# marcin-ochman/modular-slam

Hardware: AMD Instinct MI355X
Metric: ORB keypoints extracted+matched /sec, 640×480 RGB-D, 1/2/4/8 GPU; HBM GB/s vs roofline (higher is better)
Workload: dtype u8

## Files before the change

### include/mslam_hip.h

```cpp
#ifndef MSLAM_HIP_H_
#define MSLAM_HIP_H_

#include <stddef.h>
#include <stdint.h>

#ifdef __cplusplus
extern "C" {
#endif

#define MSLAM_HIP_ABI_VERSION 5

enum
{
    MSLAM_HIP_OK = 0,
    MSLAM_HIP_E_INVALID = 1,
    MSLAM_HIP_E_RUNTIME = 2,
    MSLAM_HIP_E_CAPACITY = 3,
    MSLAM_HIP_E_NO_VOCABULARY = 4,
    MSLAM_HIP_E_FORMAT = 5,
    MSLAM_HIP_E_NO_MODEL = 6
};

typedef struct mslam_hip_ctx mslam_hip_ctx;

// ... 412 lines not shown
                               const double* tvec, int min_matched_points, int new_keyframe_min_landmarks, int new_id,
                               double z_max, mslam_hip_track_window_result* out , int* first_event,
                               int32_t* vote_counts, int32_t* entry_src, int32_t* entry_kp, int entry_capacity);

#define MSLAM_HIP_TSDF_CHUNK 64
#define MSLAM_HIP_TSDF_MAX_VOXELS (1 << 30)
#define MSLAM_HIP_TSDF_MAX_FRAMES 32768
typedef struct
{
    int32_t nx, ny, nz;
    int32_t max_frames;
    double voxel;
    double origin[3];
    double trunc;
    double max_depth;
    int32_t width, height;
    float factor;
    int32_t reserved;
    double fx, fy, cx, cy;
} mslam_hip_tsdf_params;
int mslam_hip_tsdf_create(mslam_hip_ctx* ctx, const mslam_hip_tsdf_params* params);
int mslam_hip_tsdf_destroy(mslam_hip_ctx* ctx);
int mslam_hip_tsdf_info(mslam_hip_ctx* ctx, mslam_hip_tsdf_params* out , int* n_frames );
int mslam_hip_tsdf_add_frame(mslam_hip_ctx* ctx, int frame_id, const uint16_t* depth, const double* R, const double* t);
int mslam_hip_tsdf_add_frame_dev(mslam_hip_ctx* ctx, int frame_id, const uint16_t* d_depth, const double* R, const double* t);
int mslam_hip_tsdf_get_frame(mslam_hip_ctx* ctx, int frame_id, double* R, double* t);
int mslam_hip_tsdf_update_poses(mslam_hip_ctx* ctx, const int32_t* frame_ids, const double* R ,
                                const double* t , int n, int* n_moved);
int mslam_hip_tsdf_remove_frame(mslam_hip_ctx* ctx, int frame_id);
int mslam_hip_tsdf_read(mslam_hip_ctx* ctx, int32_t* S, int32_t* W);
int mslam_hip_tsdf_extract(mslam_hip_ctx* ctx, int min_weight, float* xyz, float* normal, int capacity, int* n);

typedef struct
{
    int32_t width, height;
    double fx, fy, cx, cy;
    double z_near, z_far, step;
    int32_t coarse;
    int32_t min_weight;
} mslam_hip_tsdf_raycast_params;
int mslam_hip_tsdf_raycast(mslam_hip_ctx* ctx, const mslam_hip_tsdf_raycast_params* params, const double* R, const double* t,
                           float* depth, float* xyz, float* normal, int* n_hits);
int mslam_hip_tsdf_raycast_dev(mslam_hip_ctx* ctx, const mslam_hip_tsdf_raycast_params* params, const double* R, const double* t,
                               float* d_depth, float* d_xyz, float* d_normal, int* n_hits);

enum
{
    MSLAM_HIP_DBG_PYRAMID = 0,
    MSLAM_HIP_DBG_BLURRED = 1,
    MSLAM_HIP_DBG_CANDIDATES = 2,
    MSLAM_HIP_DBG_SELECTED = 3,
    MSLAM_HIP_DBG_CELLS = 4,
    MSLAM_HIP_DBG_FORMS = 5,
    MSLAM_HIP_DBG_QUAD_DIRECT = 6
};
int mslam_hip_level_geometry(mslam_hip_ctx* ctx, int* widths, int* heights, float* scales);
int mslam_hip_debug_read(mslam_hip_ctx* ctx, int what, int frame, int level, void* dst, size_t dst_bytes,
                         size_t* n_items);

int mslam_hip_debug_counts(mslam_hip_ctx* ctx, int what, int32_t* out, int n_frames);

int mslam_hip_copy_to_host(mslam_hip_ctx* ctx, void* dst_host, const void* src_dev, size_t bytes);

int mslam_hip_set_profiling(mslam_hip_ctx* ctx, int enable);
int mslam_hip_get_stage_times(mslam_hip_ctx* ctx, const char** names, float* ms, int cap, int* n);

#ifdef __cplusplus
}
#endif
#endif
```

### modular-slam_amd/__init__.py

```python
import contextlib
import ctypes as C
import os
import subprocess

import numpy as np

_HERE = os.path.dirname(os.path.abspath(__file__))
LIB_PATH = os.path.join(_HERE, "libmslam_hip.so")

OK, E_INVALID, E_RUNTIME, E_CAPACITY, E_NO_VOCABULARY, E_FORMAT, E_NO_MODEL = range(7)
DBG_PYRAMID, DBG_BLURRED, DBG_CANDIDATES, DBG_SELECTED, DBG_CELLS, DBG_FORMS, DBG_QUAD_DIRECT = range(7)
QUAD_DIRECT_MAX_CANDIDATES = 1024
MATCHER_AUTO, MATCHER_POPCOUNT = 0, 1
DETECTOR_DISTRIBUTED, DETECTOR_CV_ORB = 0, 1
BOW_ASSIGN_TREE, BOW_ASSIGN_FLAT = 0, 1
CV_ORDER_LIBSTDCXX, CV_ORDER_RASTER = 0, 1
POSE_GRAPH_MAX_KEYFRAMES, POSE_GRAPH_MAX_EDGES = 1024, 65536
POSE_GRAPH_MAX_KEYFRAMES_SPARSE, POSE_GRAPH_MAX_ENVELOPE_BLOCKS = 16384, 1048576
PG_SOLVER_DENSE, PG_SOLVER_SPARSE = 0, 1
_PG_SOLVER_NAMES = {"dense": PG_SOLVER_DENSE, "sparse": PG_SOLVER_SPARSE}
PG_ORDER_NATURAL, PG_ORDER_RCM = 0, 1
BA_GLOBAL_MAX_KEYFRAMES, BA_GLOBAL_MAX_KEYFRAMES_SPARSE = 1024, 16384
BA_GLOBAL_SOLVER_DENSE, BA_GLOBAL_SOLVER_SPARSE = 0, 1
BA_GLOBAL_PCG_MAX_ITERATIONS, BA_GLOBAL_PCG_TOLERANCE = 500, 1e-6
POSE_GRAPH_PCG_MAX_ITERATIONS, POSE_GRAPH_PCG_TOLERANCE = 500, 1e-6
CULL_MAX_ENTRIES = 4096
BA_LOSS_NONE, BA_LOSS_HUBER, BA_LOSS_CAUCHY = 0, 1, 2
_BA_LOSS_NAMES = {"none": BA_LOSS_NONE, "huber": BA_LOSS_HUBER, "cauchy": BA_LOSS_CAUCHY}
UNION_DESC_RECENT, UNION_DESC_DISTINCTIVE = 0, 1
_UNION_DESC_NAMES = {"recent": UNION_DESC_RECENT, "distinctive": UNION_DESC_DISTINCTIVE}
TRACK_POSE_PNP, TRACK_POSE_ALIGN = 0, 1
_TRACK_POSE_NAMES = {"pnp": TRACK_POSE_PNP, "align": TRACK_POSE_ALIGN}
TSDF_CHUNK, TSDF_MAX_VOXELS, TSDF_MAX_FRAMES = 64, 1 << 30, 32768

ABI_SYMBOLS = [
    "mslam_hip_default_params", "mslam_hip_abi_version", "mslam_hip_create", "mslam_hip_destroy",
    "mslam_hip_last_error", "mslam_hip_sync", "mslam_hip_detect", "mslam_hip_detect_batch_dev",
    "mslam_hip_get_batch_view", "mslam_hip_match", "mslam_hip_match_knn2", "mslam_hip_match_batch_dev",
    "mslam_hip_bow_load", "mslam_hip_bow_info", "mslam_hip_bow_words", "mslam_hip_bow_transform",
    "mslam_hip_bow_score", "mslam_hip_bow_db_add", "mslam_hip_bow_db_query", "mslam_hip_bow_db_clear",
    "mslam_hip_bow_batch_dev", "mslam_hip_get_bow_view", "mslam_hip_bow_cross_score_dev", "mslam_hip_level_geometry", "mslam_hip_debug_read",
    "mslam_hip_set_profiling", "mslam_hip_get_stage_times", "mslam_hip_copy_to_host", "mslam_hip_backproject", "mslam_hip_backproject_batch_dev",
    "mslam_hip_get_points_view", "mslam_hip_set_matcher", "mslam_hip_get_matcher",
    "mslam_hip_bow_pack_dev", "mslam_hip_bow_cross_score_packed_dev", "mslam_hip_debug_counts",
    "mslam_hip_last_match_kernel",
    "mslam_hip_join_matcher", "mslam_hip_bow_db_remove", "mslam_hip_bow_set_assignment",
    "mslam_hip_bow_db_reserve", "mslam_hip_bow_db_size", "mslam_hip_qlz_decompress",
    "mslam_hip_pnp_ransac", "mslam_hip_pnp_batch_dev", "mslam_hip_get_pnp_view", "mslam_hip_pnp_set_confidence", "mslam_hip_pack_batch_dev", "mslam_hip_packed_capacity",
    "mslam_hip_set_cv_keypoint_order", "mslam_hip_pnp_min_mse", "mslam_hip_pnp_min_mse_batch_dev",
    "mslam_hip_kf_add", "mslam_hip_kf_add_from_batch_dev", "mslam_hip_kf_remove", "mslam_hip_kf_clear", "mslam_hip_kf_size",
    "mslam_hip_kf_reserve", "mslam_hip_kf_read", "mslam_hip_relocalize",
    "mslam_hip_kf_visible", "mslam_hip_track", "mslam_hip_track_window", "mslam_hip_track_window_dev",
    "mslam_hip_kf_add_ids", "mslam_hip_kf_read_ids", "mslam_hip_kf_covisible", "mslam_hip_kf_union", "mslam_hip_kf_union_dev",
    "mslam_hip_match_guided_knn2", "mslam_hip_match_guided", "mslam_hip_set_guided_match", "mslam_hip_get_guided_match",
    "mslam_hip_bundle_adjust", "mslam_hip_bundle_adjust_global", "mslam_hip_kf_update_world", "mslam_hip_pose_graph",
    "mslam_hip_kf_fuse_search", "mslam_hip_kf_replace_ids", "mslam_hip_kf_fuse",
    "mslam_hip_kf_fuse_search_multi", "mslam_hip_kf_fuse_multi",
    "mslam_hip_kf_remove_observations",
    "mslam_hip_kf_observers", "mslam_hip_kf_cull_search", "mslam_hip_kf_cull",
    "mslam_hip_kf_remove_landmarks", "mslam_hip_kf_cull_landmarks_search", "mslam_hip_kf_cull_landmarks",
    "mslam_hip_set_ba_loss", "mslam_hip_get_ba_loss",
    "mslam_hip_set_union_descriptor", "mslam_hip_get_union_descriptor",
    "mslam_hip_set_pose_graph_solver", "mslam_hip_get_pose_graph_solver", "mslam_hip_pose_graph_analyze",
    "mslam_hip_set_ba_global_solver", "mslam_hip_get_ba_global_solver", "mslam_hip_bundle_adjust_global_analyze",
    "mslam_hip_set_pose_graph_loss", "mslam_hip_get_pose_graph_loss", "mslam_hip_pose_graph_edge_weights",
# ... 1215 lines not shown
    def bow_pack_dev(self, k_max, d_out):
        self._chk(self.L.mslam_hip_bow_pack_dev(self._h, int(k_max), C.c_void_p(d_out)))

    def bow_cross_score_packed_dev(self, d_sets, n_sets, self_set, n_frames, k_max, d_scores, stream=None):
        self._chk(self.L.mslam_hip_bow_cross_score_packed_dev(self._h, C.c_void_p(d_sets), int(n_sets), int(self_set),
                                                              int(n_frames), int(k_max), C.c_void_p(d_scores),
                                                              C.c_void_p(stream)))

    def bow_view(self):
        v = BowView()
        self._chk(self.L.mslam_hip_get_bow_view(self._h, C.byref(v)))
        return v

    def level_geometry(self):
        n = self.params.n_levels
        w = (C.c_int * 16)()
        h = (C.c_int * 16)()
        s = (C.c_float * 16)()
        self._chk(self.L.mslam_hip_level_geometry(self._h, w, h, s))
        return list(w[:n]), list(h[:n]), np.array(s[:n], np.float32)

    def debug_image(self, what, frame, level):
        w, h, _ = self.level_geometry()
        out = np.empty((h[level], w[level]), np.uint8)
        n = C.c_size_t(0)
        self._chk(self.L.mslam_hip_debug_read(self._h, what, frame, level, _p(out), C.c_size_t(out.size), C.byref(n)))
        return out

    def debug_keypoints(self, what, frame, level):
        out = np.empty((self.params.max_candidates, 3), np.float32)
        n = C.c_size_t(0)
        self._chk(self.L.mslam_hip_debug_read(self._h, what, frame, level, _p(out), C.c_size_t(out.nbytes),
                                              C.byref(n)))
        return out[:n.value].copy()

    def debug_cells(self, level):
        out = np.empty((2048, 6), np.int32)
        n = C.c_size_t(0)
        self._chk(self.L.mslam_hip_debug_read(self._h, DBG_CELLS, 0, level, _p(out), C.c_size_t(out.nbytes),
                                              C.byref(n)))
        return out[:n.value].copy()

    def debug_forms(self):
        out = np.zeros(2, np.int32)
        n = C.c_size_t(0)
        self._chk(self.L.mslam_hip_debug_read(self._h, DBG_FORMS, 0, 0, _p(out), C.c_size_t(out.nbytes), C.byref(n)))
        return int(out[0]), int(out[1])

    def debug_quad_direct_levels(self):
        out = np.zeros(1, np.uint32)
        n = C.c_size_t(0)
        self._chk(self.L.mslam_hip_debug_read(self._h, DBG_QUAD_DIRECT, 0, 0, _p(out), C.c_size_t(out.nbytes), C.byref(n)))
        return [bool((int(out[0]) >> l) & 1) for l in range(self.params.n_levels)]

    def debug_counts(self, what, n_frames):
        out = np.zeros((max(n_frames, 1), self.params.n_levels), np.int32)
        self._chk(self.L.mslam_hip_debug_counts(self._h, int(what), _p(out), int(out.shape[0])))
        return out[:n_frames]

    def set_profiling(self, enable):
        self._chk(self.L.mslam_hip_set_profiling(self._h, int(enable)))

    def stage_times(self, cap=256):
        names = (C.c_char_p * cap)()
        ms = (C.c_float * cap)()
        n = C.c_int(0)
        self._chk(self.L.mslam_hip_get_stage_times(self._h, names, ms, cap, C.byref(n)))
        return [(names[i].decode(), ms[i]) for i in range(n.value)]


def qlz_decompress(data, n_packets, capacity=None):
    src = np.frombuffer(bytes(data), np.uint8)
    cap = capacity if capacity is not None else 10000 * n_packets + 16
    dst = np.empty(max(cap, 1), np.uint8)
    n = C.c_size_t(0)
    L = lib()
    L.mslam_hip_qlz_decompress.argtypes = [C.c_void_p, C.c_size_t, C.c_uint32, C.c_void_p, C.c_size_t, C.POINTER(C.c_size_t)]
    rc = L.mslam_hip_qlz_decompress(_p(src), src.size, int(n_packets), _p(dst), dst.size, C.byref(n))
    if rc != OK:
        raise MslamHipError(rc, "qlz_decompress failed")
    return dst[:n.value].tobytes()


class RgbFrame:

    def __init__(self, data, width, height):
        self.data = np.ascontiguousarray(data, np.uint8).reshape(height, width, 3)
        self.size = (width, height)


class OrbKeypoint:
    __slots__ = ("id", "coordinates", "descriptor")

    def __init__(self, id, coordinates, descriptor):
        self.id, self.coordinates, self.descriptor = id, coordinates, descriptor


class HipOrbDetector:

    def __init__(self, width=640, height=480, **kw):
        self.ctx = Context(width=width, height=height, **kw)

    def detect(self, sensorData):
        r = self.ctx.detect(sensorData.data)
        return [OrbKeypoint(i, (float(x), float(y)), d) for i, ((x, y), d) in enumerate(zip(r["xy"].astype(np.float64),
                                                                                          r["desc"]))]
# ... 953 lines not shown
```

### modular-slam_amd/csrc/api.hip

```cpp
#include "context.hpp"

#include <cfloat>
#include <climits>
#include <cmath>
#include <cstdio>
#include <cstring>
#include <cstdlib>
#include <algorithm>

using namespace mslam;

static thread_local std::string g_create_error;

#define ENTER(c)                                                                                                       \
    do                                                                                                                 \
    {                                                                                                                  \
        if(!(c))                                                                                                       \
            return MSLAM_HIP_E_INVALID;                                                                                \
        MSLAM_CHK(c, hipSetDevice((c)->p.device));                                                                     \
    } while(0)

static inline int cv_round_f(float v) { return (int)lrintf(v); }
static inline int cv_floor_f(float v)
{
// ... 621 lines not shown
            const char* k = getenv("MSLAM_HIP_LEVEL_K6");
            const char* ks = getenv("MSLAM_HIP_LEVEL_K6_SMALL");
            c->level_k6_small = ks ? std::max(0, atoi(ks)) : 0;
            {
                const char* lc = getenv("MSLAM_HIP_LEVEL_CHAIN");
                const char* lf = getenv("MSLAM_HIP_LEVEL_CHAIN_FRAMES");
                const char* lw = getenv("MSLAM_HIP_LEVEL_CHAIN_WAVES");
                const char* lk = getenv("MSLAM_HIP_LEVEL_CHAIN_K6");
                c->level_chain = lc ? atoi(lc) : 0;
                c->level_chain_frames = lf ? std::max(1, std::min(64, atoi(lf))) : 2;
                c->level_chain_waves = lw ? atoi(lw) : 8;
                if(c->level_chain_waves != 4)
                    c->level_chain_waves = 8;
                c->level_chain_k6 = lk ? std::max(1, std::min(9, atoi(lk))) : 9;
            }
            c->level_k6 = k ? std::max(1, atoi(k)) : 5;
            const bool fits = (p.width & 3) == 0 && (double)B * p.width * p.height * 3 < 4294967296.0 &&
                              (double)B * g.slab < 4294901760.0  && (size_t)B * (p.width / 4) < (1u << 22) && p.height >= 8;
            int n_fused = fits ? 1 : 0;
            while(n_fused >= 1 && n_fused < p.n_levels && c->rs_q[n_fused] != SIZE_MAX && g.lv[n_fused].h >= 8 &&
                  (size_t)B * ((g.lv[n_fused].w + 3) / 4) < (1u << 22))
                ++n_fused;
            c->fused_levels = std::max(0, std::min(want, n_fused));
            const char* t = getenv("MSLAM_HIP_TILED_BLUR");
            c->geom.blur_tiled = c->fused_levels == p.n_levels && !(t && atoi(t) == 0) ? 1 : 0;
        }
        std::vector<BlurWave> bw;
        build_blur_waves(g, c->fused_levels, bw);
        c->blur_wpf = (int)bw.size();
        if(!bw.empty())
        {
            MSLAM_CHK(c, c->d_blur_waves.alloc(bw.size()));
            MSLAM_CHK(c, hipMemcpy(c->d_blur_waves, bw.data(), bw.size() * sizeof(BlurWave), hipMemcpyHostToDevice));
        }
    }
    MSLAM_CHK(c, c->d_cell_cnt.alloc(B * g.n_cells));
    MSLAM_CHK(c, c->d_cell_kp.alloc(B * g.n_cells * (size_t)kCellCap));
    QuadArgs& q = c->quad;
    MSLAM_CHK(c, c->q_cand.alloc(B * L * cap));
    MSLAM_CHK(c, c->q_cand_cnt.alloc(B * L));
    MSLAM_CHK(c, c->q_sel.alloc(B * L * cap));
    MSLAM_CHK(c, c->q_sel_cnt.alloc(B * L));
    MSLAM_CHK(c, c->q_kp_node.alloc(B * L * cap));
    MSLAM_CHK(c, c->q_nodes_a.alloc(B * L * cap));
    MSLAM_CHK(c, c->q_nodes_b.alloc(B * L * cap));
    MSLAM_CHK(c, c->q_ncnt_a.alloc(B * L * cap));
    MSLAM_CHK(c, c->q_ncnt_b.alloc(B * L * cap));
    MSLAM_CHK(c, c->q_child_cnt.alloc(B * L * cap * 4));
    MSLAM_CHK(c, c->q_ninfo.alloc(B * L * cap));
    MSLAM_CHK(c, c->q_best.alloc(B * L * cap));
    q.cand = c->q_cand, q.cand_cnt = c->q_cand_cnt, q.sel = c->q_sel, q.sel_cnt = c->q_sel_cnt, q.kp_node = c->q_kp_node;
    q.nodes_a = c->q_nodes_a, q.nodes_b = c->q_nodes_b, q.ncnt_a = c->q_ncnt_a, q.ncnt_b = c->q_ncnt_b;
    q.child_cnt = c->q_child_cnt, q.ninfo = c->q_ninfo, q.best = c->q_best;
    q.cell_cnt = c->d_cell_cnt;
    q.cell_kp = c->d_cell_kp;
    q.flags = c->d_flags;
    q.cand_cap = p.max_candidates;
    q.min_size = p.min_node_area;
    }

    for(auto& o : c->out)
    {
        MSLAM_CHK(c, o.xy.alloc((B + 1) * K * 2));
        MSLAM_CHK(c, o.desc.alloc((B + 1) * K * 32));
        MSLAM_CHK(c, o.octave.alloc((B + 1) * K));
        MSLAM_CHK(c, o.angle.alloc((B + 1) * K));
        MSLAM_CHK(c, o.response.alloc((B + 1) * K));
        MSLAM_CHK(c, o.count.alloc(B + 1));
        MSLAM_CHK(c, hipMemset(o.count, 0, (B + 1) * 4));
        MSLAM_CHK(c, o.idx0.alloc(B * K));
        MSLAM_CHK(c, o.idx1.alloc(B * K));
        MSLAM_CHK(c, o.dist0.alloc(B * K));
        MSLAM_CHK(c, o.dist1.alloc(B * K));
        MSLAM_CHK(c, o.mfrom.alloc(B * K));
        MSLAM_CHK(c, o.mto.alloc(B * K));
        MSLAM_CHK(c, o.mcount.alloc(B));
        MSLAM_CHK(c, hipMemset(o.mcount, 0, B * 4));
        MSLAM_CHK(c, hipEventCreateWithFlags(&o.ev_detect, hipEventDisableTiming));
        MSLAM_CHK(c, hipEventCreateWithFlags(&o.ev_match, hipEventDisableTiming));
    }
    MSLAM_CHK(c, hipStreamCreateWithFlags(&c->stream_m, hipStreamNonBlocking));
    {
        const char* e = getenv("MSLAM_HIP_OVERLAP_MATCH");
        c->overlap_match = !(e && atoi(e) == 0);
        auto on = [](const char* name) { const char* v = getenv(name); return !v || atoi(v) != 0; };
        c->knob_mirror_results = on("MSLAM_HIP_MIRROR_RESULTS");
        c->knob_zero_copy = on("MSLAM_HIP_ZERO_COPY_FRAME");
        c->knob_match_graph = on("MSLAM_HIP_MATCH_GRAPH");
        const char* zm = getenv("MSLAM_HIP_ZERO_COPY_MAX_BYTES");
        c->zero_copy_max_bytes = zm ? (size_t)atoll(zm) : (size_t)1200000;
        const char* m = getenv("MSLAM_HIP_MATCHER");
        c->matcher_kind = (m && std::strcmp(m, "popcount") == 0) ? MSLAM_HIP_MATCHER_POPCOUNT : MSLAM_HIP_MATCHER_AUTO;
    }
    c->cur = 0;
    MSLAM_CHK(c, hipDeviceSynchronize());
    return MSLAM_HIP_OK;
}

int mslam_hip_create(const mslam_hip_params* p, mslam_hip_ctx** out)
{
    if(!p || !out)
    {
        g_create_error = "null argument";
        return MSLAM_HIP_E_INVALID;
    }
    *out = nullptr;
// ... 261 lines not shown
                if(l < c->fused_levels)
                {
                    enqueue_resize_blur(c, l, c->d_rs_ofs + c->rs_y[l], c->d_rs_coef + c->rs_y[l], 0, f0, nf, k6_batch, cs);
                    continue;
                }
                if(c->rs_q[l] != SIZE_MAX)
                {
                    const LevelGeom &sl = g.lv[l - 1], &dl = g.lv[l];
                    ResizeColArgs ra{};
                    ra.pyr = c->d_pyr;
                    ra.slab = g.slab;
                    ra.src_off = sl.offset;
                    ra.sh = sl.h;
                    ra.spitch = sl.pitch;
                    ra.dst_off = dl.offset;
                    ra.dw = dl.w;
                    ra.dh = dl.h;
                    ra.dpitch = dl.pitch;
                    ra.qt = c->d_rs_qt + 3 * c->rs_q[l];
                    ra.yofs = c->d_rs_ofs + c->rs_y[l];
                    ra.ycoef = c->d_rs_coef + c->rs_y[l];
                    ra.frame0 = f0;
                    ra.n_frames = nf;
                    ra.quads = (dl.w + 3) / 4;
                    ra.inv_quads = 1.0f / (float)ra.quads;
                    ra.R = 8;
                    ra.need_mask = c->rs_need[l];
                    launch_resize_col(ra, cs);
                }
                else
                    launch_resize(c->d_pyr, g, l, c->d_rs_ofs + c->rs_x[l], c->d_rs_coef + c->rs_x[l],
                                  c->d_rs_ofs + c->rs_y[l], c->d_rs_coef + c->rs_y[l], f0, nf, cs);
            }
        }
        {
            StageScope t(c, "fast", cs);
            launch_fast(c->d_pyr, g, c->d_cells, c->d_cell_cnt, c->d_cell_kp, c->p.ini_fast_thr, c->p.min_fast_thr, f0,
                        nf, cs);
        }
        const bool blur_needed = c->fused_levels < g.n_levels;
        const bool forked = c->fork_blur && !c->profiling && blur_needed;
        if(forked)
        {
            MSLAM_CHK(c, hipEventRecord(c->ev_blur_fork[k], cs));
            MSLAM_CHK(c, hipStreamWaitEvent(c->blur_stream[k], c->ev_blur_fork[k], 0));
            {
                StageScope t(c, "blur", c->blur_stream[k]);
                launch_blur(c->d_pyr, c->d_blur, g, c->d_blur_waves, c->blur_wpf, f0, nf, c->blur_stream[k]);
            }
            MSLAM_CHK(c, hipEventRecord(c->ev_blur_join[k], c->blur_stream[k]));
        }
        {
            StageScope t(c, "quadtree", cs);
            launch_quadtree(g, c->quad, f0, nf, cs);
        }
        if(forked)
            MSLAM_CHK(c, hipStreamWaitEvent(cs, c->ev_blur_join[k], 0));
        else if(blur_needed)
        {
            StageScope t(c, "blur", cs);
            launch_blur(c->d_pyr, c->d_blur, g, c->d_blur_waves, c->blur_wpf, f0, nf, cs);
        }
        }
        if(cv_mode && c->fused_levels < g.n_levels)
        {
            StageScope t(c, "blur", cs);
            launch_blur(c->d_pyr, c->d_blur, g, c->d_blur_waves, c->blur_wpf, f0, nf, cs);
        }
        {
            StageScope t(c, "describe", cs);
            DescArgs a{};
            a.pyr = c->d_pyr;
            a.blur = c->d_blur;
            a.sel = c->quad.sel;
            a.sel_cnt = c->quad.sel_cnt;
            a.orient_w = c->d_orient_w;
            a.cand_cap = c->p.max_candidates;
            a.max_kp = c->p.max_keypoints;
            a.xy = cur_out(c).xy + K * 2;
            a.desc = cur_out(c).desc + K * 32;
            a.octave = cur_out(c).octave + K;
            a.angle = cur_out(c).angle + K;
            a.response = cur_out(c).response + K;
            a.count = cur_out(c).count + 1;
            a.flags = c->d_flags;
            if(cv_mode)
            {
                a.sel_resp = reinterpret_cast<const float*>(c->quad.best);
                a.cv_mode = 1;
            }
            if(c->mirror_results && n_frames == 1)
                a.h_mirror = c->h_out.dev();
            launch_describe(g, a, f0, nf, cs);
        }
        if(n_chunks > 1)
        {
            MSLAM_CHK(c, hipEventRecord(c->ev_join[k], cs));
            MSLAM_CHK(c, hipStreamWaitEvent(s, c->ev_join[k], 0));
        }
    }
    MSLAM_CHK(c, hipGetLastError());
    return MSLAM_HIP_OK;
}

static int detect_prologue(mslam_hip_ctx* c)
{
    const size_t K = (size_t)c->p.max_keypoints;
// ... 568 lines not shown
        for(uint32_t i = 0; i < n; ++i)
        {
            out[3 * i] = (float)kp_x(tmp[i]);
            out[3 * i + 1] = (float)kp_y(tmp[i]);
            out[3 * i + 2] = (float)kp_score(tmp[i]);
        }
        if(c->p.detector == MSLAM_HIP_DETECTOR_CV_ORB && !cand)
        {
            std::vector<float> resp(n);
            if(n)
                MSLAM_CHK(c, hipMemcpy(resp.data(), reinterpret_cast<const float*>(c->quad.best) + slot * (size_t)c->p.max_candidates,
                                       (size_t)n * 4, hipMemcpyDeviceToHost));
            for(uint32_t i = 0; i < n; ++i)
            {
                out[3 * i] += (float)kBorder;
                out[3 * i + 1] += (float)kBorder;
                out[3 * i + 2] = resp[i];
            }
        }
        return MSLAM_HIP_OK;
    }
    if(what == MSLAM_HIP_DBG_CELLS && c->p.detector == MSLAM_HIP_DETECTOR_DISTRIBUTED)
    {
        *n_items = (size_t)lv.n_cells;
        if(dst_bytes < (size_t)lv.n_cells * 24)
            return fail(c, MSLAM_HIP_E_CAPACITY, "debug_read: buffer too small");
        int32_t* out = static_cast<int32_t*>(dst);
        for(int i = 0; i < lv.n_cells; ++i)
        {
            const CellDesc& cd = c->cells[(size_t)lv.cell_base + i];
            const int32_t rec[6] = {cd.x0, cd.y0, cd.cw, cd.ch, cd.ox, cd.oy};
            std::memcpy(out + 6 * i, rec, sizeof(rec));
        }
        return MSLAM_HIP_OK;
    }
    if(what == MSLAM_HIP_DBG_FORMS)
    {
        *n_items = 2;
        if(dst_bytes < 8)
            return fail(c, MSLAM_HIP_E_CAPACITY, "debug_read: buffer too small");
        const int32_t rec[2] = {c->fused_levels, c->geom.blur_tiled};
        std::memcpy(dst, rec, sizeof(rec));
        return MSLAM_HIP_OK;
    }
    if(what == MSLAM_HIP_DBG_QUAD_DIRECT)
    {
        *n_items = 1;
        if(dst_bytes < 4)
            return fail(c, MSLAM_HIP_E_CAPACITY, "debug_read: buffer too small");
        const uint32_t m = c->p.detector == MSLAM_HIP_DETECTOR_DISTRIBUTED ? quad_direct_levels(c->geom) : 0u;
        std::memcpy(dst, &m, sizeof(m));
        return MSLAM_HIP_OK;
    }
    return fail(c, MSLAM_HIP_E_INVALID, "debug_read: unknown item");
}

int mslam_hip_debug_counts(mslam_hip_ctx* c, int what, int32_t* out, int n_frames)
{
    ENTER(c);
    if(c->p.width == 0 || !out || n_frames < 1 || (what != MSLAM_HIP_DBG_CANDIDATES && what != MSLAM_HIP_DBG_SELECTED))
        return fail(c, MSLAM_HIP_E_INVALID, "debug_counts: bad argument");
    MSLAM_CHK(c, hipStreamSynchronize(c->stream));
    const int rows = std::min(n_frames, std::max(c->n_last, 1));
    MSLAM_CHK(c, hipMemcpy(out, what == MSLAM_HIP_DBG_CANDIDATES ? c->quad.cand_cnt : c->quad.sel_cnt,
                           (size_t)rows * c->geom.n_levels * 4, hipMemcpyDeviceToHost));
    return MSLAM_HIP_OK;
}

int mslam_hip_copy_to_host(mslam_hip_ctx* c, void* dst_host, const void* src_dev, size_t bytes)
{
    ENTER(c);
    if(!dst_host || !src_dev)
        return fail(c, MSLAM_HIP_E_INVALID, "copy_to_host: null pointer");
    MSLAM_CHK(c, hipStreamSynchronize(c->stream_m));
    MSLAM_CHK(c, hipStreamSynchronize(c->stream));
    MSLAM_CHK(c, hipMemcpy(dst_host, src_dev, bytes, hipMemcpyDeviceToHost));
    return MSLAM_HIP_OK;
}

int mslam_hip_set_profiling(mslam_hip_ctx* c, int enable)
{
    if(!c)
        return MSLAM_HIP_E_INVALID;
    c->profiling = enable == 1;
    c->inplace_timing = enable == 2;
    c->timers_used = 0;
    return MSLAM_HIP_OK;
}

int mslam_hip_get_stage_times(mslam_hip_ctx* c, const char** names, float* ms, int cap, int* n)
{
    ENTER(c);
    if(!n)
        return fail(c, MSLAM_HIP_E_INVALID, "get_stage_times: null output");
    MSLAM_CHK(c, hipStreamSynchronize(c->stream_m));
    MSLAM_CHK(c, hipStreamSynchronize(c->stream));
    int k = 0;
    for(size_t i = 0; i < c->timers_used && k < cap; ++i, ++k)
    {
        float t = 0;
        MSLAM_CHK(c, hipEventElapsedTime(&t, c->timers[i].start, c->timers[i].stop));
        if(names)
            names[k] = c->timers[i].name;
        if(ms)
            ms[k] = t;
    }
// ... 8 lines not shown
```

### modular-slam_amd/csrc/common.hpp

```cpp
#pragma once
#include <hip/hip_runtime.h>
#include <cstdint>
#include <cstddef>

namespace mslam
{

constexpr int kMaxLevels = 16;
constexpr int kBorder = 19;
constexpr int kCell = 64;
constexpr int kOverlap = 6;
constexpr int kCellCap = 1024;

constexpr size_t al256(size_t x) { return (x + 255) & ~(size_t)255; }

struct LevelGeom
{
    int w, h;
    int pitch;
    int offset;
    float scale;
    int bw, bh;
    int cell_base;
    int n_cells;
// ... 50 lines not shown

enum : uint32_t
{
    kFlagCandOverflow = 1u,
    kFlagKpOverflow = 2u,
    kFlagQuadNoConverge = 4u,
    kFlagBowPackOverflow = 8u,
    kFlagDbFull = 16u,
    kFlagPackOverflow = 32u,
    kFlagUnionOverflow = 64u
};

void launch_gray(const uint8_t* d_bgr, uint8_t* d_pyr, const Geometry& g, int frame0, int n_frames, hipStream_t s);
void launch_resize(uint8_t* d_pyr, const Geometry& g, int level, const int32_t* d_xofs, const uint32_t* d_xcoef,
                   const int32_t* d_yofs, const uint32_t* d_ycoef, int frame0, int n_frames, hipStream_t s);
struct ResizeColArgs
{
    uint8_t* pyr;
    unsigned slab;
    int src_off, sh, spitch, dst_off, dw, dh, dpitch;
    const uint4* qt;
    const int32_t* yofs;
    const uint32_t* ycoef;
    int frame0, n_frames;
    int quads;
    float inv_quads;
    int R;
    int need_mask;
    int exact;
};
void launch_resize_col(const ResizeColArgs& a, hipStream_t s);
void launch_fast(const uint8_t* d_pyr, const Geometry& g, const CellDesc* d_cells, uint32_t* d_cell_cnt,
                 uint32_t* d_cell_kp, int ini_thr, int min_thr, int frame0, int n_frames, hipStream_t s);
void launch_denorm_selfcheck(uint32_t* d_out, hipStream_t s);
struct QuadArgs
{
    const uint32_t* cell_cnt;
    const uint32_t* cell_kp;
    uint32_t* cand;
    uint32_t* cand_cnt;
    uint32_t* sel;
    uint32_t* sel_cnt;
    uint32_t* kp_node;
    uint2* nodes_a;
    uint2* nodes_b;
    uint32_t* ncnt_a;
    uint32_t* ncnt_b;
    uint32_t* child_cnt;
    uint32_t* ninfo;
    uint32_t* best;
    uint32_t* flags;
    int cand_cap;
    unsigned min_size;
};
void launch_quadtree(const Geometry& g, const QuadArgs& a, int frame0, int n_frames, hipStream_t s);
int quad_depth_bound(const LevelGeom& lv, unsigned min_size);
unsigned quad_direct_levels(const Geometry& g);
struct BlurK
{
    uint32_t ta[3], tb[4], tc[4];
    uint32_t t01, t23, t45, t6;
};
BlurK make_blur_k();
struct GrayBlurArgs
{
    const uint8_t* bgr;
    uint8_t* pyr;
    uint8_t* blur;
    int W, H, pitch;
    unsigned slab;
    int n_frames, frame0;
    int quads;
    float inv_quads;
    int wide;
    int k6;
    int waves_per_xcd;
    int blur_tiled;
    BlurK bk;
};
void launch_gray_blur(const GrayBlurArgs& a, hipStream_t s);
struct ResizeBlurArgs
{
    uint8_t* pyr;
    uint8_t* blur;
    unsigned slab;
    int src_off, sh, spitch, dst_off, dw, dh, dpitch;
    const uint4* qt;
    const int32_t* yofs;
    const uint32_t* ycoef;
    int frame0, n_frames;
    int quads;
    float inv_quads;
    int wide;
    int k6;
    int need_mask;
    int exact;
    int waves_per_xcd;
    int blur_tiled;
    int always_load;
    BlurK bk;
};
void launch_resize_blur(const ResizeBlurArgs& a, hipStream_t s);
constexpr int kOctNeed = 0x48;
constexpr int kChainLevels = 8;
struct LevelChainArgs
{
    GrayBlurArgs g;
    ResizeBlurArgs lv[kChainLevels - 1];
    int n_lv;
    int G;
// ... 163 lines not shown
```

### modular-slam_amd/csrc/context.hpp

```cpp
#pragma once
#include "common.hpp"
#include "devmem.hpp"
#include "../../include/mslam_hip.h"
#include <array>
#include <string>
#include <vector>

namespace mslam
{
struct BowState;
void bow_destroy(BowState*);
struct RelocState;
void reloc_destroy(RelocState*);
struct TsdfState;
void tsdf_destroy(TsdfState*);
void set_blur_taps(const int* taps);
void build_blur_waves(const Geometry& g, int first_level, std::vector<BlurWave>& out);

struct StageTimer
{
    const char* name;
    hipEvent_t start, stop;
};
}
// ... 17 lines not shown
    mslam::Geometry geom{};
    hipStream_t stream = nullptr;
    bool own_stream = false;
    int n_side = 2;
    hipStream_t side[4] = {nullptr, nullptr, nullptr, nullptr};
    hipEvent_t ev_fork = nullptr, ev_join[4] = {nullptr, nullptr, nullptr, nullptr};
    hipStream_t blur_stream[4] = {nullptr, nullptr, nullptr, nullptr};
    hipEvent_t ev_blur_fork[4] = {nullptr, nullptr, nullptr, nullptr}, ev_blur_join[4] = {nullptr, nullptr, nullptr, nullptr};
    bool fork_blur = false;
    std::string err;

    std::vector<mslam::CellDesc> cells;

    mslam::DevBuf<mslam::CellDesc> d_cells;
    mslam::DevBuf<int32_t> d_rs_ofs;
    mslam::DevBuf<uint32_t> d_rs_coef;
    std::vector<size_t> rs_x, rs_y;
    mslam::DevBuf<uint4> d_rs_qt;
    std::vector<size_t> rs_q;
    std::vector<int> rs_need;
    mslam::DevBuf<uint4> d_rs_qt8;
    std::vector<size_t> rs_q8;
    mslam::DevBuf<int32_t> d_cv_ofs;
    mslam::DevBuf<uint32_t> d_cv_coef;
    std::vector<size_t> cv_x, cv_y;
    std::vector<std::array<int, 4>> cv_range;
    std::vector<int> cv_window12;
    int cv_quota[mslam::kMaxLevels] = {0};
    mslam::DevBuf<int32_t> d_ratio_thr;
    mslam::DevBuf<uint32_t> d_orient_w;
    hipGraphExec_t detect_graph[2] = {nullptr, nullptr};
    bool use_graph = true;
    int cv_order = 0;
    bool mirror_results = false;
    hipGraphExec_t match_graph = nullptr;
    int match_graph_from_cap = 0, match_graph_to_cap = 0, match_graph_kind = -1, match_graph_kernel = 0;
    mslam::PinnedBuf<uint8_t> h_out;
    double ratio_cached = -1.0;

    mslam::DevBuf<uint8_t> d_stage;
    mslam::PinnedBuf<uint8_t> h_stage;
    mslam::DevBuf<uint8_t> d_pyr, d_blur;
    mslam::DevBuf<mslam::BlurWave> d_blur_waves;
    int blur_wpf = 0;
    int fused_levels = 0;
    int level_k6 = 5;
    bool knob_mirror_results = true, knob_zero_copy = true, knob_match_graph = true;
    size_t zero_copy_max_bytes = 1200000;
    int level_chain = 0, level_chain_frames = 2, level_chain_waves = 8, level_chain_k6 = 9;
    int level_k6_small = 1;
    mslam::DevBuf<uint32_t> d_cell_cnt, d_cell_kp;
    mslam::DevBuf<uint32_t> q_cand, q_cand_cnt, q_sel, q_sel_cnt, q_kp_node, q_ncnt_a, q_ncnt_b, q_child_cnt, q_ninfo, q_best;
    mslam::DevBuf<uint2> q_nodes_a, q_nodes_b;
    mslam::QuadArgs quad{};
    mslam::DevBuf<uint32_t> d_flags;

    mslam_out_set out[2];
    int cur = 0;
    hipStream_t stream_m = nullptr;
    bool overlap_match = true;
    int matcher_kind = 0;
    int last_match_kernel = 0;
    double guided_radius = 0.0;
    int guided_max_distance = 256, guided_width = 0, guided_height = 0;
    int union_descriptor = MSLAM_HIP_UNION_DESC_RECENT;
    int n_last = 0;
    unsigned long long detect_seq = 0;
    unsigned long long points_seq = ~0ull;
    unsigned long long match_seq = ~0ull;
    bool have_prev = false;

    mslam::DevBuf<uint8_t> d_hm_from;
    uint8_t* d_hm_to = nullptr;
    mslam::DevBuf<int32_t> d_hm_out;
    int hm_from_cap = 0, hm_to_cap = 0;
    mslam::DevBuf<uint32_t> d_hm_partial;
    mslam::PinnedBuf<uint8_t> h_hm;

    mslam::DevBuf<double> d_xyz;
    mslam::DevBuf<uint8_t> d_valid;
    mslam::DevBuf<float> d_pnp_obj, d_pnp_img;
    mslam::DevBuf<int32_t> d_pnp_n, d_pnp_counts;
    mslam::DevBuf<double> d_pnp_hyp, d_pnp_out;
    mslam::DevBuf<uint8_t> d_pnp_mask;
    int pnp_iterations = 0;
    double pnp_confidence = 0.99;
    int ba_loss_kind = MSLAM_HIP_BA_LOSS_NONE;
    double ba_loss_scale = 0.0;
    mslam::DevBuf<float> d_pnp1_obj, d_pnp1_img;
    mslam::DevBuf<double> d_pnp1_hyp, d_pnp1_out;
    mslam::DevBuf<int32_t> d_pnp1_counts;
    mslam::DevBuf<uint8_t> d_pnp1_mask;
    int pnp1_n_cap = 0, pnp1_it_cap = 0;
    mslam::DevBuf<double> d_mse1;
    mslam::DevBuf<float> d_align1_src, d_align1_dst;
    mslam::DevBuf<double> d_align1_hyp, d_align1_out;
    mslam::DevBuf<int32_t> d_align1_counts;
    mslam::DevBuf<uint8_t> d_align1_mask;
    int align1_n_cap = 0, align1_it_cap = 0;
    mslam::DevBuf<float> d_align_src, d_align_dst;
    mslam::DevBuf<int32_t> d_align_n, d_align_counts;
    mslam::DevBuf<double> d_align_hyp, d_align_out;
    mslam::DevBuf<uint8_t> d_align_mask;
    int align_iterations = 0;
    int track_pose_kind = MSLAM_HIP_TRACK_POSE_PNP;
    double track_align_distance = 0.0;
// ... 121 lines not shown
```

### modular-slam_amd/csrc/k_quadtree.hip

```cpp
#include "common.hpp"
#include <algorithm>
#include <cstdlib>

namespace mslam
{

constexpr int QT = 512;
constexpr int kSmallKp = 512, kSmallQT = 256;
constexpr int kMidKp = 1024, kMidQT = 512;
constexpr int kLdsKp = 2048;
constexpr int kMaxCellsPerLevel = 2048;
constexpr int kBigNodes = 4096;
constexpr int kBigKp = 12288;
constexpr int kBigMinPixels = 400000;
constexpr int kMaxInitNodes = 64;
constexpr int kDirectKp = 1024, kDirectQT = 256, kDirectSlots = 1365, kDirectMaxDepth = 10;
constexpr int kMaxPasses = 40;

struct Scan
{
    uint32_t wsum[QT / 64];
};

__device__ __forceinline__ uint32_t wave_incl_scan(uint32_t v)
// ... 466 lines not shown
                              a.nodes_a + slot * cap, a.nodes_b + slot * cap, a.ncnt_a + slot * cap,
                              a.ncnt_b + slot * cap, a.ninfo + slot * cap, a.best + slot * cap,
                              a.child_cnt + slot * cap * 4, a.best + slot * cap, sel, scan, scan2, init_cnt, init_pos,
                              sh_n);
    }
}

template <int SLOTS>
struct DirectTable
{
    uint32_t cnt[(SLOTS + 1) / 2];
    uint32_t best[SLOTS];
    uint8_t flag[SLOTS];
};

__device__ __forceinline__ uint32_t direct_block_start(uint32_t n_init, int d) { return n_init * (((1u << (2 * d)) - 1u) / 3u); }

template <int KP, int SLOTS, int NT>
__global__ __launch_bounds__(NT) __attribute__((amdgpu_waves_per_eu(8))) void k_quadtree_direct(Geometry g, QuadArgs a, unsigned direct_levels)
{
    constexpr int PER = KP / NT;
    static_assert(KP % NT == 0 && KP == kDirectKp, "instance shape");
    __shared__ Scan scan;
    __shared__ uint32_t l_cand[KP];
    __shared__ DirectTable<SLOTS> t;
    __shared__ uint32_t tot[2 * (kDirectMaxDepth + 2)];

    const int level = (int)((blockIdx.x + blockIdx.y) % (unsigned)g.n_levels);
    if(!((direct_levels >> level) & 1u))
        return;
    const size_t frame = blockIdx.y + g.frame0;
    const LevelGeom& lv = g.lv[level];
    const int tid = threadIdx.x;
    const size_t slot = frame * g.n_levels + level;
    const size_t cap = (size_t)a.cand_cap;
    uint32_t* g_cand = a.cand + slot * cap;
    uint32_t* sel = a.sel + slot * cap;
    const int D = lv.qdepth;
    const uint32_t n_init = (uint32_t)(lv.nxg * lv.nyg);
    const uint32_t n_slots = direct_block_start(n_init, D + 1);

    for(uint32_t i = tid; i < (n_slots + 1) / 2; i += NT)
        t.cnt[i] = 0;
    for(uint32_t i = tid; i < n_slots; i += NT)
        t.flag[i] = 0;
    if(tid < 2 * (kDirectMaxDepth + 2))
        tot[tid] = 0;

    const int n_cells = lv.n_cells;
    uint32_t* cell_off = t.best;
    const uint32_t* ccnt = a.cell_cnt + frame * g.n_cells + lv.cell_base;
    const uint32_t N = quad_cell_offsets<NT>(ccnt, n_cells, cell_off, scan);
    if(N > (uint32_t)KP)
        return;
    if(N > (uint32_t)a.cand_cap)
    {
        if(tid == 0)
        {
            atomicOr(a.flags, kFlagCandOverflow);
            a.cand_cnt[slot] = 0;
            a.sel_cnt[slot] = 0;
        }
        return;
    }
    if(tid == 0)
        a.cand_cnt[slot] = N;
    if(N == 0)
    {
        if(tid == 0)
            a.sel_cnt[slot] = 0;
        return;
    }

    const uint32_t* ckp = a.cell_kp + (frame * g.n_cells + lv.cell_base) * (size_t)kCellCap;
    const float sf = lv.scale;
    const float min_size_f = (float)a.min_size;
    uint32_t path[PER];
#pragma unroll
    for(int i = 0; i < PER; ++i)
    {
        const uint32_t k = (uint32_t)(tid + i * NT);
        path[i] = ~0u;
        if(k >= N)
            continue;
        int lo = 0, hi = n_cells - 1;
        while(lo < hi)
        {
            const int mid = (lo + hi + 1) >> 1;
            if(cell_off[mid] <= k)
                lo = mid;
            else
                hi = mid - 1;
        }
        const uint32_t p = ckp[(size_t)lo * kCellCap + (k - cell_off[lo])];
        l_cand[k] = p;
        g_cand[k] = p;
        const int x = kp_x(p), y = kp_y(p);
        const unsigned ix = (unsigned)((double)(float)x / lv.delta_x);
        const unsigned iy = (unsigned)((double)(float)y / lv.delta_y);
        const unsigned idx = ix + iy * (unsigned)lv.nxg;
        if(idx >= n_init)
            continue;
        int bx = (int)(lv.delta_x * ix), by = (int)(lv.delta_y * iy);
        int ex = (int)(lv.delta_x * (ix + 1)), ey = (int)(lv.delta_y * (iy + 1));
        uint32_t q = idx;
        int d = 0;
        for(;;)
// ... 63 lines not shown
        const int last = dk < top ? dk : top;
        uint32_t leaf = 0;
        for(int d = 0; d <= last; ++d)
        {
            leaf = direct_block_start(n_init, d) + (q >> (2 * (dk - d)));
            if(t.flag[leaf] == 1)
                break;
        }
        atomicMax(&t.best[leaf], ((uint32_t)kp_score(l_cand[k]) << 24) | (0xFFFFFFu - k));
    }
    __syncthreads();

    const uint32_t n_entries = direct_block_start(n_init, top + 1);
    const uint32_t per = (n_entries + NT - 1) / NT;
    const uint32_t e0 = (uint32_t)tid * per, e1 = e0 + per < n_entries ? e0 + per : n_entries;
    auto entry_slot = [&](uint32_t e, bool& is_leaf) {
        int d = top;
        uint32_t n_d = n_init << (2 * d);
        while(e >= n_d)
        {
            e -= n_d;
            --d;
            n_d >>= 2;
        }
        const uint32_t bits = 2u * (uint32_t)d, low_mask = (1u << bits) - 1u;
        uint32_t i0 = e >> bits;
        if(d & 1)
            i0 = n_init - 1u - i0;
        const uint32_t s = direct_block_start(n_init, d) + ((i0 << bits) | ((e ^ 0x33333333u) & low_mask));
        const uint32_t f = t.flag[s];
        is_leaf = f == 1 || (f == 2 && d == P);
        return s;
    };
    uint32_t mine = 0;
    for(uint32_t e = e0; e < e1; ++e)
    {
        bool is_leaf;
        entry_slot(e, is_leaf);
        mine += is_leaf ? 1u : 0u;
    }
    uint32_t n_leaves;
    uint32_t r = block_excl_scan<NT>(mine, scan, n_leaves);
    for(uint32_t e = e0; e < e1 && mine != 0; ++e)
    {
        bool is_leaf;
        const uint32_t s = entry_slot(e, is_leaf);
        if(is_leaf)
            sel[r++] = l_cand[0xFFFFFFu - (t.best[s] & 0xFFFFFFu)];
    }
    if(tid == 0)
        a.sel_cnt[slot] = n_leaves;
}

unsigned quad_direct_levels(const Geometry& g)
{
    const char* env = getenv("MSLAM_HIP_QUAD_DIRECT");
    const bool on = !env || atoi(env) != 0;
    unsigned m = 0;
    for(int l = 0; on && l < g.n_levels; ++l)
    {
        const LevelGeom& lv = g.lv[l];
        if(lv.qdepth < 0 || lv.qdepth > kDirectMaxDepth || lv.n_cells + 1 > kDirectSlots)
            continue;
        const long long slots = (long long)lv.nxg * lv.nyg * (((1ll << (2 * (lv.qdepth + 1))) - 1) / 3);
        if(slots <= kDirectSlots)
            m |= 1u << l;
    }
    return m;
}

int quad_depth_bound(const LevelGeom& lv, unsigned min_size)
{
    int dx = 0, dy = 0;
    for(int iy = 0; iy < lv.nyg; ++iy)
        for(int ix = 0; ix < lv.nxg; ++ix)
        {
            dx = std::max(dx, (int)(lv.delta_x * (ix + 1)) - (int)(lv.delta_x * ix));
            dy = std::max(dy, (int)(lv.delta_y * (iy + 1)) - (int)(lv.delta_y * iy));
        }
    for(int d = 0; d <= 15; ++d)
    {
        const unsigned area = (unsigned)(dx * dy);
        const float scaled = (float)area * lv.scale;
        if(scaled * lv.scale <= (float)min_size)
            return d;
        if(dx <= 1 && dy <= 1)
            break;
        dx = (dx + 1) >> 1, dy = (dy + 1) >> 1;
    }
    return -1;
}

void launch_quadtree(const Geometry& g, const QuadArgs& a, int frame0, int n_frames, hipStream_t s)
{
    dim3 grid(g.n_levels, n_frames);
    Geometry gg = g;
    gg.frame0 = frame0;
    unsigned big_levels = 0;
    for(int l = 0; l < g.n_levels; ++l)
        if(g.lv[l].w * g.lv[l].h > kBigMinPixels)
            big_levels |= 1u << l;
    static const unsigned classes_env = [] { const char* e = getenv("MSLAM_HIP_QUAD_CLASSES"); return e ? (unsigned)atoi(e) & 3u : 3u; }();
    const unsigned direct = quad_direct_levels(g);
    const bool all_direct = direct == (g.n_levels >= 32 ? ~0u : (1u << g.n_levels) - 1u);
    const unsigned classes = n_frames < 8 || all_direct ? 0u : classes_env;
    const unsigned bl = big_levels | (classes << 30);
    if(direct != 0)
        hipLaunchKernelGGL((k_quadtree_direct<kDirectKp, kDirectSlots, kDirectQT>), grid, dim3(kDirectQT), 0, s, gg, a, direct);
    hipLaunchKernelGGL((k_quadtree<kLdsKp, QT, 2>), grid, dim3(QT), 0, s, gg, a, bl, direct);
    if(classes & 2u)
        hipLaunchKernelGGL((k_quadtree<kMidKp, kMidQT, 1>), grid, dim3(kMidQT), 0, s, gg, a, bl, direct);
    if(classes & 1u)
        hipLaunchKernelGGL((k_quadtree<kSmallKp, kSmallQT, 0>), grid, dim3(kSmallQT), 0, s, gg, a, bl, direct);
    if(big_levels != 0)
    {
        constexpr size_t lds = (size_t)kBigNodes * (8 + 8 + 8 + 2 + 2 + 2 + 1) + (size_t)kBigKp * 2;
        static const bool attr = [] {
            return hipFuncSetAttribute((const void*)k_quadtree_big, hipFuncAttributeMaxDynamicSharedMemorySize, (int)lds) == hipSuccess;
        }();
        (void)attr;
        hipLaunchKernelGGL(k_quadtree_big, dim3((unsigned)__builtin_popcount(big_levels), n_frames), dim3(QT), lds, s, gg, a,
                           big_levels);
    }
}

}
```

Baseline: 668.3 million.

## Compact quadtree overflow slots into a worklist processed by a persistent rest kernel

When every level takes the direct quadtree path, the direct kernel now appends the slots it cannot handle (too many keypoints) to a global worklist through an atomic counter. A grid-strided persistent kernel then processes only those listed slots, replacing the full (levels × frames) launch of the fallback kernel whose blocks mostly exited early. The intent is to cut wasted block launches and LDS-heavy occupancy for empty work. The cost is an extra atomic counter reset protocol, per-chunk control buffers, and reliance on correct reset by the last block.

```diff
diff --git a/include/mslam_hip.h b/include/mslam_hip.h
--- a/include/mslam_hip.h
+++ b/include/mslam_hip.h
@@ -488,7 +488,8 @@
     MSLAM_HIP_DBG_SELECTED = 3,
     MSLAM_HIP_DBG_CELLS = 4,
     MSLAM_HIP_DBG_FORMS = 5,
-    MSLAM_HIP_DBG_QUAD_DIRECT = 6
+    MSLAM_HIP_DBG_QUAD_DIRECT = 6,
+    MSLAM_HIP_DBG_QUAD_REST = 7
 };
 int mslam_hip_level_geometry(mslam_hip_ctx* ctx, int* widths, int* heights, float* scales);
 int mslam_hip_debug_read(mslam_hip_ctx* ctx, int what, int frame, int level, void* dst, size_t dst_bytes,
diff --git a/modular-slam_amd/__init__.py b/modular-slam_amd/__init__.py
--- a/modular-slam_amd/__init__.py
+++ b/modular-slam_amd/__init__.py
@@ -9,8 +9,9 @@
 LIB_PATH = os.path.join(_HERE, "libmslam_hip.so")
 
 OK, E_INVALID, E_RUNTIME, E_CAPACITY, E_NO_VOCABULARY, E_FORMAT, E_NO_MODEL = range(7)
-DBG_PYRAMID, DBG_BLURRED, DBG_CANDIDATES, DBG_SELECTED, DBG_CELLS, DBG_FORMS, DBG_QUAD_DIRECT = range(7)
+DBG_PYRAMID, DBG_BLURRED, DBG_CANDIDATES, DBG_SELECTED, DBG_CELLS, DBG_FORMS, DBG_QUAD_DIRECT, DBG_QUAD_REST = range(8)
 QUAD_DIRECT_MAX_CANDIDATES = 1024
+QUAD_REST_GRID = 512
 MATCHER_AUTO, MATCHER_POPCOUNT = 0, 1
 DETECTOR_DISTRIBUTED, DETECTOR_CV_ORB = 0, 1
 BOW_ASSIGN_TREE, BOW_ASSIGN_FLAT = 0, 1
@@ -1332,6 +1333,12 @@
         n = C.c_size_t(0)
         self._chk(self.L.mslam_hip_debug_read(self._h, DBG_QUAD_DIRECT, 0, 0, _p(out), C.c_size_t(out.nbytes), C.byref(n)))
         return [bool((int(out[0]) >> l) & 1) for l in range(self.params.n_levels)]
+
+    def debug_quad_rest_list(self):
+        out = np.zeros(1, np.uint32)
+        n = C.c_size_t(0)
+        self._chk(self.L.mslam_hip_debug_read(self._h, DBG_QUAD_REST, 0, 0, _p(out), C.c_size_t(out.nbytes), C.byref(n)))
+        return bool(out[0])
 
     def debug_counts(self, what, n_frames):
         out = np.zeros((max(n_frames, 1), self.params.n_levels), np.int32)
diff --git a/modular-slam_amd/csrc/api.hip b/modular-slam_amd/csrc/api.hip
--- a/modular-slam_amd/csrc/api.hip
+++ b/modular-slam_amd/csrc/api.hip
@@ -697,6 +697,10 @@
     q.cand = c->q_cand, q.cand_cnt = c->q_cand_cnt, q.sel = c->q_sel, q.sel_cnt = c->q_sel_cnt, q.kp_node = c->q_kp_node;
     q.nodes_a = c->q_nodes_a, q.nodes_b = c->q_nodes_b, q.ncnt_a = c->q_ncnt_a, q.ncnt_b = c->q_ncnt_b;
     q.child_cnt = c->q_child_cnt, q.ninfo = c->q_ninfo, q.best = c->q_best;
+    MSLAM_CHK(c, c->q_rest_list.alloc((size_t)kQuadRestChunks * B * L));
+    MSLAM_CHK(c, c->q_rest_ctl.alloc((size_t)kQuadRestChunks * kQuadRestCtlStride));
+    MSLAM_CHK(c, hipMemset(c->q_rest_ctl, 0, (size_t)kQuadRestChunks * kQuadRestCtlStride * 4));
+    q.rest_list = c->q_rest_list, q.rest_ctl = c->q_rest_ctl, q.rest_cap = (uint32_t)(B * L);
     q.cell_cnt = c->d_cell_cnt;
     q.cell_kp = c->d_cell_kp;
     q.flags = c->d_flags;
@@ -1064,7 +1068,7 @@
         }
         {
             StageScope t(c, "quadtree", cs);
-            launch_quadtree(g, c->quad, f0, nf, cs);
+            launch_quadtree(g, c->quad, f0, nf, k, cs);
         }
         if(forked)
             MSLAM_CHK(c, hipStreamWaitEvent(cs, c->ev_blur_join[k], 0));
@@ -1739,6 +1743,15 @@
         std::memcpy(dst, &m, sizeof(m));
         return MSLAM_HIP_OK;
     }
+    if(what == MSLAM_HIP_DBG_QUAD_REST)
+    {
+        *n_items = 1;
+        if(dst_bytes < 4)
+            return fail(c, MSLAM_HIP_E_CAPACITY, "debug_read: buffer too small");
+        const uint32_t m = c->p.detector == MSLAM_HIP_DETECTOR_DISTRIBUTED && quad_rest_list(c->geom, c->quad) ? 1u : 0u;
+        std::memcpy(dst, &m, sizeof(m));
+        return MSLAM_HIP_OK;
+    }
     return fail(c, MSLAM_HIP_E_INVALID, "debug_read: unknown item");
 }
 
diff --git a/modular-slam_amd/csrc/common.hpp b/modular-slam_amd/csrc/common.hpp
--- a/modular-slam_amd/csrc/common.hpp
+++ b/modular-slam_amd/csrc/common.hpp
@@ -126,10 +126,17 @@
     uint32_t* flags;
     int cand_cap;
     unsigned min_size;
-};
-void launch_quadtree(const Geometry& g, const QuadArgs& a, int frame0, int n_frames, hipStream_t s);
+    uint32_t* rest_list;
+    uint32_t* rest_ctl;
+    uint32_t rest_cap;
+};
+constexpr int kQuadRestChunks = 4;
+constexpr int kQuadRestCtlStride = 32;
+constexpr int kQuadRestGrid = 512;
+void launch_quadtree(const Geometry& g, const QuadArgs& a, int frame0, int n_frames, int chunk, hipStream_t s);
 int quad_depth_bound(const LevelGeom& lv, unsigned min_size);
 unsigned quad_direct_levels(const Geometry& g);
+bool quad_rest_list(const Geometry& g, const QuadArgs& a);
 struct BlurK
 {
     uint32_t ta[3], tb[4], tc[4];
diff --git a/modular-slam_amd/csrc/context.hpp b/modular-slam_amd/csrc/context.hpp
--- a/modular-slam_amd/csrc/context.hpp
+++ b/modular-slam_amd/csrc/context.hpp
@@ -93,6 +93,7 @@
     mslam::DevBuf<uint32_t> d_cell_cnt, d_cell_kp;
     mslam::DevBuf<uint32_t> q_cand, q_cand_cnt, q_sel, q_sel_cnt, q_kp_node, q_ncnt_a, q_ncnt_b, q_child_cnt, q_ninfo, q_best;
     mslam::DevBuf<uint2> q_nodes_a, q_nodes_b;
+    mslam::DevBuf<uint32_t> q_rest_list, q_rest_ctl;
     mslam::QuadArgs quad{};
     mslam::DevBuf<uint32_t> d_flags;
 
diff --git a/modular-slam_amd/csrc/k_quadtree.hip b/modular-slam_amd/csrc/k_quadtree.hip
--- a/modular-slam_amd/csrc/k_quadtree.hip
+++ b/modular-slam_amd/csrc/k_quadtree.hip
@@ -542,7 +542,15 @@
     const uint32_t* ccnt = a.cell_cnt + frame * g.n_cells + lv.cell_base;
     const uint32_t N = quad_cell_offsets<NT>(ccnt, n_cells, cell_off, scan);
     if(N > (uint32_t)KP)
-        return;
+    {
+        if(a.rest_ctl != nullptr && tid == 0)
+        {
+            const uint32_t i = atomicAdd(&a.rest_ctl[0], 1u);
+            if(i < a.rest_cap)
+                a.rest_list[i] = (uint32_t)slot;
+        }
+        return;
+    }
     if(N > (uint32_t)a.cand_cap)
     {
         if(tid == 0)
@@ -712,6 +720,73 @@
         a.sel_cnt[slot] = n_leaves;
 }
 
+__global__ __launch_bounds__(QT) __attribute__((amdgpu_waves_per_eu(4))) void k_quadtree_rest(Geometry g, QuadArgs a, unsigned big_levels)
+{
+    constexpr int KP = kLdsKp;
+    __shared__ Scan scan, scan2;
+    __shared__ uint32_t l_cand[KP];
+    __shared__ uint2 l_nodes_a[KP], l_nodes_b[KP];
+    __shared__ uint32_t l_cc[KP * 2];
+    __shared__ uint16_t l_kp_node[KP], l_ncnt_a[KP], l_ncnt_b[KP], l_nbase[KP];
+    __shared__ uint8_t l_ninfo[KP];
+    __shared__ uint32_t init_cnt[kMaxInitNodes];
+    __shared__ uint32_t init_pos[kMaxInitNodes];
+    __shared__ uint32_t sh_n, sh_entries;
+    static_assert(2 * KP - 1 >= kMaxCellsPerLevel, "cell offsets must fit");
+    uint32_t* cell_off = reinterpret_cast<uint32_t*>(l_nodes_b);
+    const int tid = threadIdx.x;
+
+    if(tid == 0)
+    {
+        unsigned long long* ctl = reinterpret_cast<unsigned long long*>(a.rest_ctl);
+        const unsigned long long old = atomicAdd(ctl, 1ull << 32);
+        if((uint32_t)(old >> 32) == gridDim.x - 1u)
+            __hip_atomic_store(ctl, 0ull, __ATOMIC_RELAXED, __HIP_MEMORY_SCOPE_AGENT);
+        const uint32_t n = (uint32_t)old;
+        sh_entries = n < a.rest_cap ? n : a.rest_cap;
+    }
+    __syncthreads();
+    const uint32_t n_entries = sh_entries;
+    const size_t cap = (size_t)a.cand_cap;
+    for(uint32_t e = blockIdx.x; e < n_entries; e += gridDim.x)
+    {
+        if(e != blockIdx.x)
+            __syncthreads();
+        const size_t slot = a.rest_list[e];
+        const size_t frame = slot / (unsigned)g.n_levels;
+        const int level = (int)(slot % (unsigned)g.n_levels);
+        const LevelGeom& lv = g.lv[level];
+        uint32_t* cand = a.cand + slot * cap;
+        uint32_t* sel = a.sel + slot * cap;
+        const int n_cells = lv.n_cells;
+        const uint32_t* ccnt = a.cell_cnt + frame * g.n_cells + lv.cell_base;
+        const uint32_t N = quad_cell_offsets<QT>(ccnt, n_cells, cell_off, scan);
+        if(N > (uint32_t)a.cand_cap)
+        {
+            if(tid == 0)
+            {
+                atomicOr(a.flags, kFlagCandOverflow);
+                a.cand_cnt[slot] = 0;
+                a.sel_cnt[slot] = 0;
+            }
+            continue;
+        }
+        if(tid == 0)
+            a.cand_cnt[slot] = N;
+        if(N <= (uint32_t)KP)
+            quad_run<LdsStore, QT>(g, a, lv, frame, slot, tid, N, n_cells, cell_off, l_cand, cand, l_kp_node, l_nodes_a, l_nodes_b,
+                                   l_ncnt_a, l_ncnt_b, l_ninfo, l_nbase, l_cc, l_cc, sel, scan, scan2, init_cnt, init_pos, sh_n);
+        else if((big_levels >> level) & 1u)
+            continue;
+        else
+            quad_run<GlobalStore, QT>(g, a, lv, frame, slot, tid, N, n_cells, cell_off, cand, cand, a.kp_node + slot * cap,
+                                      a.nodes_a + slot * cap, a.nodes_b + slot * cap, a.ncnt_a + slot * cap,
+                                      a.ncnt_b + slot * cap, a.ninfo + slot * cap, a.best + slot * cap,
+                                      a.child_cnt + slot * cap * 4, a.best + slot * cap, sel, scan, scan2, init_cnt, init_pos,
+                                      sh_n);
+    }
+}
+
 unsigned quad_direct_levels(const Geometry& g)
 {
     const char* env = getenv("MSLAM_HIP_QUAD_DIRECT");
@@ -727,6 +802,14 @@
             m |= 1u << l;
     }
     return m;
+}
+
+bool quad_rest_list(const Geometry& g, const QuadArgs& a)
+{
+    const char* env = getenv("MSLAM_HIP_QUAD_REST_LIST");
+    if((env && atoi(env) == 0) || a.rest_ctl == nullptr || a.rest_list == nullptr)
+        return false;
+    return quad_direct_levels(g) == (g.n_levels >= 32 ? ~0u : (1u << g.n_levels) - 1u);
 }
 
 int quad_depth_bound(const LevelGeom& lv, unsigned min_size)
@@ -751,8 +834,9 @@
     return -1;
 }
 
-void launch_quadtree(const Geometry& g, const QuadArgs& a, int frame0, int n_frames, hipStream_t s)
-{
+void launch_quadtree(const Geometry& g, const QuadArgs& args, int frame0, int n_frames, int chunk, hipStream_t s)
+{
+    QuadArgs a = args;
     dim3 grid(g.n_levels, n_frames);
     Geometry gg = g;
     gg.frame0 = frame0;
@@ -765,9 +849,24 @@
     const bool all_direct = direct == (g.n_levels >= 32 ? ~0u : (1u << g.n_levels) - 1u);
     const unsigned classes = n_frames < 8 || all_direct ? 0u : classes_env;
     const unsigned bl = big_levels | (classes << 30);
+    const bool rest_list = all_direct && chunk >= 0 && chunk < kQuadRestChunks && quad_rest_list(g, a);
+    if(rest_list)
+    {
+        a.rest_list += (size_t)chunk * a.rest_cap;
+        a.rest_ctl += (size_t)chunk * kQuadRestCtlStride;
+    }
+    else
+        a.rest_ctl = nullptr;
     if(direct != 0)
         hipLaunchKernelGGL((k_quadtree_direct<kDirectKp, kDirectSlots, kDirectQT>), grid, dim3(kDirectQT), 0, s, gg, a, direct);
-    hipLaunchKernelGGL((k_quadtree<kLdsKp, QT, 2>), grid, dim3(QT), 0, s, gg, a, bl, direct);
+    if(rest_list)
+    {
+        const char* rg = getenv("MSLAM_HIP_QUAD_REST_GRID");
+        const int G = rg ? std::max(1, std::min(atoi(rg), 4096)) : kQuadRestGrid;
+        hipLaunchKernelGGL(k_quadtree_rest, dim3((unsigned)std::min(G, g.n_levels * n_frames)), dim3(QT), 0, s, gg, a, big_levels);
+    }
+    else
+        hipLaunchKernelGGL((k_quadtree<kLdsKp, QT, 2>), grid, dim3(QT), 0, s, gg, a, bl, direct);
     if(classes & 2u)
         hipLaunchKernelGGL((k_quadtree<kMidKp, kMidQT, 1>), grid, dim3(kMidQT), 0, s, gg, a, bl, direct);
     if(classes & 1u)
```

Result: no change. 673.9 million (median of 6 runs) (+0.8%).
